# Kelvin-ywc/LPI

Hardware: AMD Instinct MI355X
Metric: image-text pairs/sec fwd+bwd (ViT-B/16, bs256/GPU) (higher is better)
Workload: dtype bf16; 1 GPU; BASELINE.json configs[2]: ViT-B/16 dual encoder bs=256/GPU prompt_depth=3 r=4 P=16, fwd+bwd incl. DecomposedPrompt grads + SGD step; global_batch=256, image=224x224, towers=lock step, GEMMs of one layer op grouped in one launch, parallelism=dp1, weights=synthetic (numpy Philox, CLIP-init scales), frozen

## Files before the change

lpi_amd/csrc/attention.hip:

```cpp
#include <type_traits>
#include "common.h"
#include "attn_softmax.h"

extern int g_lpi_tuning[16];

namespace {

constexpr int HD = 64;
constexpr int NB = 2;
constexpr float LOG2E = 1.4426950408889634f;
constexpr float LN2 = 0.6931471805599453f;
constexpr float SCALE = 0.125f;

template <typename T> struct AT;
template <> struct AT<float> {
    static constexpr int KS = 4;
    static constexpr int RS = 272;
};
template <> struct AT<f16_t> {
    static constexpr int KS = 2;
    static constexpr int RS = 160;
};
template <> struct AT<bf16_t> {
    static constexpr int KS = 2;
    static constexpr int RS = 160;
};

template <typename T, bool CV0 = false, bool CV1 = false, bool SW = false>
__device__ __forceinline__ void stage_rows2(char* lds0, const T* g0, char* lds1, const T* g1, int ld0, int ld1, int L, int Lp, int pre = 0, long seg = 0) {
    constexpr int NCH = HD * (int)sizeof(T) / 16;
    const int n = Lp * NCH, nt = blockDim.x;
    for (int base = threadIdx.x; base < n; base += 4 * nt) {
        uint4 v0[4], v1[4];
#pragma unroll
        for (int j = 0; j < 4; ++j) {
            const int i = base + j * nt, row = i / NCH, c = i % NCH;
            v0[j] = make_uint4(0, 0, 0, 0);
            v1[j] = make_uint4(0, 0, 0, 0);
            if (i < n && row < L) {
                const size_t srow = (size_t)(row < pre ? (long)row : (long)row + seg);
                v0[j] = *reinterpret_cast<const uint4*>(g0 + srow * ld0 + c * Elem<T>::EPC);
                v1[j] = *reinterpret_cast<const uint4*>(g1 + srow * ld1 + c * Elem<T>::EPC);
            }
        }
#pragma unroll
        for (int j = 0; j < 4; ++j) {
            const int i = base + j * nt, row = i / NCH, c = i % NCH;
            if (i < n) {
                if constexpr (CV0) { Chunk t; t.u = v0[j]; chunk_f16_to_bf16(t); v0[j] = t.u; }
                if constexpr (CV1) { Chunk t; t.u = v1[j]; chunk_f16_to_bf16(t); v1[j] = t.u; }
                const int lo = SW ? row * 128 + ((c ^ (row & 6)) << 4) : row * AT<T>::RS + c * 16;
                *reinterpret_cast<uint4*>(lds0 + lo) = v0[j];
                *reinterpret_cast<uint4*>(lds1 + lo) = v1[j];
            }
        }
    }
}

template <typename T, bool CVA>
__device__ __forceinline__ void stage_rows4(char* lds_k, const T* gk, char* lds_v, const T* gv, int ldkv, int La, int pre, long seg,
                                            char* lds_q, const T* gq, int ldq, char* lds_do, const T* gdo, int lddo, int Lb, int Lp) {
    constexpr int NCH = HD * (int)sizeof(T) / 16;
    const int n = Lp * NCH, nt = blockDim.x;
    for (int base = threadIdx.x; base < n; base += 4 * nt) {
        uint4 vk[4], vv[4], vq[4], vd[4];
#pragma unroll
        for (int j = 0; j < 4; ++j) {
            const int i = base + j * nt, row = i / NCH, c = i % NCH;
            vk[j] = vv[j] = vq[j] = vd[j] = make_uint4(0, 0, 0, 0);
            if (i < n && row < La) {
                const size_t srow = (size_t)(row < pre ? (long)row : (long)row + seg);
                vk[j] = *reinterpret_cast<const uint4*>(gk + srow * ldkv + c * Elem<T>::EPC);
                vv[j] = *reinterpret_cast<const uint4*>(gv + srow * ldkv + c * Elem<T>::EPC);
            }
            if (i < n && row < Lb) {
                vq[j] = *reinterpret_cast<const uint4*>(gq + (size_t)row * ldq + c * Elem<T>::EPC);
                vd[j] = *reinterpret_cast<const uint4*>(gdo + (size_t)row * lddo + c * Elem<T>::EPC);
            }
        }
#pragma unroll
        for (int j = 0; j < 4; ++j) {
            const int i = base + j * nt, row = i / NCH, c = i % NCH;
            if (i < n) {
                if constexpr (CVA) {
                    Chunk t;
                    t.u = vk[j]; chunk_f16_to_bf16(t); vk[j] = t.u;
                    t.u = vv[j]; chunk_f16_to_bf16(t); vv[j] = t.u;
                    t.u = vq[j]; chunk_f16_to_bf16(t); vq[j] = t.u;
                }
                const int lo = row * AT<T>::RS + c * 16;
                *reinterpret_cast<uint4*>(lds_k + lo) = vk[j];
                *reinterpret_cast<uint4*>(lds_v + lo) = vv[j];
                *reinterpret_cast<uint4*>(lds_q + lo) = vq[j];
                *reinterpret_cast<uint4*>(lds_do + lo) = vd[j];
            }
        }
    }
}

template <typename T>
__device__ __forceinline__ void lds_row_chunks(Chunk (&q)[AT<T>::KS], const char* lds, int row, int grp) {
#pragma unroll
    for (int ks = 0; ks < AT<T>::KS; ++ks) q[ks].u = *reinterpret_cast<const uint4*>(lds + row * AT<T>::RS + (grp + 4 * ks) * 16);
}

template <typename T, bool CV = false>
__device__ __forceinline__ void load_row_chunks(Chunk (&q)[AT<T>::KS], const T* g, size_t row, int ld, int grp, bool valid) {
#pragma unroll
    for (int ks = 0; ks < AT<T>::KS; ++ks) {
        q[ks].u = make_uint4(0, 0, 0, 0);
        if (valid) q[ks].u = *reinterpret_cast<const uint4*>(g + row * ld + (grp + 4 * ks) * Elem<T>::EPC);
        if constexpr (CV) chunk_f16_to_bf16(q[ks]);
    }
}

__device__ __forceinline__ float fast_exp2(float x) { return __builtin_amdgcn_exp2f(x); }

typedef __attribute__((ext_vector_type(2))) float f32x2;
typedef __attribute__((ext_vector_type(2))) __bf16 bf16x2;
__device__ __forceinline__ uint32_t pack_bf16(float a, float b) {
    return __builtin_bit_cast(uint32_t, __builtin_convertvector((f32x2){a, b}, bf16x2));
}

template <typename T>
__device__ __forceinline__ void mma_lds_rows(f32x4 (&acc)[NB], const char* p, const Chunk (&b)[NB][AT<T>::KS]) {
#pragma unroll
    for (int j = 0; j < NB; ++j) acc[j] = f32x4{0.f, 0.f, 0.f, 0.f};
#pragma unroll
    for (int ks = 0; ks < AT<T>::KS; ++ks) {
        Chunk a;
        a.u = *reinterpret_cast<const uint4*>(p + ks * 64);
#pragma unroll
        for (int j = 0; j < NB; ++j) mma_chunk<T>(acc[j], a, b[j][ks]);
    }
}

template <typename T>
__device__ __forceinline__ void mma_transposed(f32x4 (&acc)[NB][4], const char* tp, const f32x4 (&p0)[NB], const f32x4 (&p1)[NB]) {
    if constexpr (sizeof(T) == 2) {
        Chunk b[NB];
#pragma unroll
        for (int j = 0; j < NB; ++j)
            b[j].u = make_uint4(pack2_t<T>(p0[j][0], p0[j][1]), pack2_t<T>(p0[j][2], p0[j][3]), pack2_t<T>(p1[j][0], p1[j][1]), pack2_t<T>(p1[j][2], p1[j][3]));
#pragma unroll
        for (int dt = 0; dt < 4; ++dt) {
            short4v lo = __builtin_amdgcn_ds_read_tr16_b64_v4i16((__attribute__((address_space(3))) short4v*)(tp + dt * 32));
            short4v hi = __builtin_amdgcn_ds_read_tr16_b64_v4i16((__attribute__((address_space(3))) short4v*)(tp + 16 * AT<T>::RS + dt * 32));
            Chunk a;
            const uint2 lo2 = __builtin_bit_cast(uint2, lo), hi2 = __builtin_bit_cast(uint2, hi);
            a.u = make_uint4(lo2.x, lo2.y, hi2.x, hi2.y);
#pragma unroll
            for (int j = 0; j < NB; ++j) mma_chunk<T>(acc[j][dt], a, b[j]);
        }
    } else {
        const float* base = reinterpret_cast<const float*>(tp);
        constexpr int RSF = AT<T>::RS / 4;
#pragma unroll
        for (int dt = 0; dt < 4; ++dt) {
            Chunk a0, a1;
#pragma unroll
            for (int s = 0; s < 4; ++s) {
                a0.f[s] = base[s * RSF + dt * 16];
                a1.f[s] = base[(16 + s) * RSF + dt * 16];
            }
#pragma unroll
            for (int j = 0; j < NB; ++j) {
                Chunk b0, b1;
                b0.f = p0[j];
                b1.f = p1[j];
                mma_chunk<T>(acc[j][dt], a0, b0);
                mma_chunk<T>(acc[j][dt], a1, b1);
            }
        }
    }
}

template <typename T>
__device__ __forceinline__ void mma_lds_rows_sw(f32x4 (&acc)[NB], const char* base, const int (&ro)[AT<T>::KS], const Chunk (&b)[NB][AT<T>::KS]) {
#pragma unroll
    for (int j = 0; j < NB; ++j) acc[j] = f32x4{0.f, 0.f, 0.f, 0.f};
#pragma unroll
    for (int ks = 0; ks < AT<T>::KS; ++ks) {
        Chunk a;
        a.u = *reinterpret_cast<const uint4*>(base + ro[ks]);
#pragma unroll
        for (int j = 0; j < NB; ++j) mma_chunk<T>(acc[j], a, b[j][ks]);
    }
}
template <typename T>
__device__ __forceinline__ void mma_transposed_sw(f32x4 (&acc)[NB][4], const char* base, const int (&to)[4], const f32x4 (&p0)[NB], const f32x4 (&p1)[NB]) {
    Chunk b[NB];
#pragma unroll
    for (int j = 0; j < NB; ++j)
        b[j].u = make_uint4(pack2_t<T>(p0[j][0], p0[j][1]), pack2_t<T>(p0[j][2], p0[j][3]), pack2_t<T>(p1[j][0], p1[j][1]), pack2_t<T>(p1[j][2], p1[j][3]));
#pragma unroll
    for (int dt = 0; dt < 4; ++dt) {
        short4v lo = __builtin_amdgcn_ds_read_tr16_b64_v4i16((__attribute__((address_space(3))) short4v*)(base + to[dt]));
        short4v hi = __builtin_amdgcn_ds_read_tr16_b64_v4i16((__attribute__((address_space(3))) short4v*)(base + 16 * 128 + to[dt]));
        Chunk a;
        const uint2 lo2 = __builtin_bit_cast(uint2, lo), hi2 = __builtin_bit_cast(uint2, hi);
        a.u = make_uint4(lo2.x, lo2.y, hi2.x, hi2.y);
#pragma unroll
        for (int j = 0; j < NB; ++j) mma_chunk<T>(acc[j][dt], a, b[j]);
    }
}

template <typename T> __device__ __forceinline__ int row_ptr_off(int lane) { return (lane & 15) * AT<T>::RS + (lane >> 4) * 16; }
template <typename T> __device__ __forceinline__ int tr_ptr_off(int lane) {
    if constexpr (sizeof(T) == 2) return (4 * (lane >> 4) + ((lane & 15) >> 2)) * AT<T>::RS + (lane & 3) * 8;
    else return 4 * (lane >> 4) * AT<T>::RS + (lane & 15) * 4;
}

__device__ __forceinline__ float group_max(float v) {
    auto r = __builtin_amdgcn_permlane16_swap(__float_as_uint(v), __float_as_uint(v), false, false);
    v = fmaxf(__uint_as_float(r[0]), __uint_as_float(r[1]));
    r = __builtin_amdgcn_permlane32_swap(__float_as_uint(v), __float_as_uint(v), false, false);
    return fmaxf(__uint_as_float(r[0]), __uint_as_float(r[1]));
}
__device__ __forceinline__ float group_sum(float v) {
    auto r = __builtin_amdgcn_permlane16_swap(__float_as_uint(v), __float_as_uint(v), false, false);
    v = __uint_as_float(r[0]) + __uint_as_float(r[1]);
    r = __builtin_amdgcn_permlane32_swap(__float_as_uint(v), __float_as_uint(v), false, false);
    return __uint_as_float(r[0]) + __uint_as_float(r[1]);
}

template <typename T, bool CAUSAL, bool SW = false>
__device__ __forceinline__ void attn_fwd_body(int bh, char* smem, int Lmax, int Lpmax, const int* __restrict__ rs, int H, const T* __restrict__ qkv, int ldqkv,
                                              T* __restrict__ ctx, int ldctx, float* __restrict__ lse, int pre = 0, int bshared = -1,
                                              int qkv_hs = 0, int qkv_vs = 0, int ctx_hs = 0) {
    const int hs = qkv_hs ? qkv_hs : HD, chs = ctx_hs ? ctx_hs : HD;
    const int b = bh / H, h = bh % H;
    int L = Lmax, Lp = Lpmax;
    size_t row0 = (size_t)b * Lmax;
    int pb = 0;
    if (CAUSAL && pre > 0 && b == bshared) {
        row0 = 0;
        L = pre;
        Lp = (L + 31) / 32 * 32;
    } else if (rs) {
        const int r = rs[b];
        row0 = (size_t)r;
        L = rs[b + 1] - r;
        if (CAUSAL && pre > 0) pb = pre;
        Lp = (pb + L + 31) / 32 * 32;
    }
    const int Lk = pb + L;
    const size_t lse0 = ((size_t)b * H + h) * Lmax;
    const int dm = qkv_vs ? qkv_vs : H * HD;
    const T* qg = qkv + row0 * ldqkv + (size_t)h * hs;
    constexpr int RSX = SW ? 128 : AT<T>::RS;
    static_assert(!SW || sizeof(T) == 2, "the swizzled images are for the 2-byte operand types");
    char* k_lds = smem;
    char* v_lds = smem + Lp * RSX;
    const int lane = threadIdx.x & 63, wave = threadIdx.x >> 6, nw = blockDim.x >> 6;
    const int g = lane >> 4;
    Chunk q[NB][AT<T>::KS];
#pragma unroll
    for (int j = 0; j < NB; ++j) {
        const int qr = (wave * NB + j) * 16 + (lane & 15);
        load_row_chunks<T>(q[j], qg, qr, ldqkv, g, qr < L);
    }
    if (pb) stage_rows2<T, false, false, SW>(k_lds, qkv + (size_t)h * hs + dm, v_lds, qkv + (size_t)h * hs + 2 * (size_t)dm, ldqkv, ldqkv, Lk, Lp, pb, (long)row0 - pb);
    else stage_rows2<T, false, false, SW>(k_lds, qg + dm, v_lds, qg + 2 * (size_t)dm, ldqkv, ldqkv, L, Lp);
    __syncthreads();

    const float c = SCALE * LOG2E;
    const char* const kp0 = k_lds + row_ptr_off<T>(lane);
    const char* const vt0 = v_lds + tr_ptr_off<T>(lane);
    int ro[AT<T>::KS], to[4];
    {
        const int r = lane & 15, rr = 4 * g + (r >> 2), pq = lane & 3;
#pragma unroll
        for (int ks = 0; ks < AT<T>::KS; ++ks) ro[ks] = r * 128 + (((g + 4 * ks) ^ (r & 6)) << 4);
#pragma unroll
        for (int dt = 0; dt < 4; ++dt) to[dt] = rr * 128 + (((2 * dt + (pq >> 1)) ^ (rr & 6)) << 4) + (pq & 1) * 8;
    }
    for (int q0 = wave * 16 * NB; q0 < L; q0 += nw * 16 * NB) {
        int qrow[NB], qpos[NB];
#pragma unroll
        for (int j = 0; j < NB; ++j) { qrow[j] = q0 + 16 * j + (lane & 15); qpos[j] = qrow[j] + pb; }
        if (q0 != wave * 16 * NB) {
#pragma unroll
            for (int j = 0; j < NB; ++j) load_row_chunks<T>(q[j], qg, qrow[j], ldqkv, g, qrow[j] < L);
        }
        float m[NB], lsum[NB];
        f32x4 o[NB][4];
#pragma unroll
        for (int j = 0; j < NB; ++j) {
            m[j] = -INFINITY;
            lsum[j] = 0.f;
#pragma unroll
            for (int i = 0; i < 4; ++i) o[j][i] = f32x4{0.f, 0.f, 0.f, 0.f};
        }
        auto tile = [&](int kb, auto masked_tag) {
            constexpr bool MASKED = decltype(masked_tag)::value;
            f32x4 s0[NB], s1[NB];
            if constexpr (SW) {
                const char* kb_ = k_lds + kb * 128;
                mma_lds_rows_sw<T>(s0, kb_, ro, q);
                mma_lds_rows_sw<T>(s1, kb_ + 16 * 128, ro, q);
                attn_softmax_tile<NB, MASKED, CAUSAL>(s0, s1, m, lsum, o, kb, g, Lk, qpos, c);
                mma_transposed_sw<T>(o, v_lds + kb * 128, to, s0, s1);
            } else {
                const char* kp = kp0 + kb * AT<T>::RS;
                mma_lds_rows<T>(s0, kp, q);
                mma_lds_rows<T>(s1, kp + 16 * AT<T>::RS, q);
                attn_softmax_tile<NB, MASKED, CAUSAL>(s0, s1, m, lsum, o, kb, g, Lk, qpos, c);
                mma_transposed<T>(o, vt0 + kb * AT<T>::RS, s0, s1);
            }
        };
        const int qlast = q0 + pb + 16 * NB - 1;
        const int kend = CAUSAL ? min(Lp, (qlast / 32 + 1) * 32) : Lp;
        const int kfull = CAUSAL ? min((Lk / 32) * 32, ((q0 + pb) / 32) * 32) : (Lk / 32) * 32;
        int kb = 0;
        for (; kb < kfull; kb += 32) tile(kb, std::false_type{});
        for (; kb < kend; kb += 32) tile(kb, std::true_type{});
#pragma unroll
        for (int j = 0; j < NB; ++j) {
            const float ltot = group_sum(lsum[j]);
            const float inv = 1.0f / ltot;
            if constexpr (sizeof(T) == 2) {
                f32x4 os[4];
#pragma unroll
                for (int dt = 0; dt < 4; ++dt) os[dt] = o[j][dt] * inv;
                store_row16_t<T>(ctx + (row0 + qrow[j]) * ldctx + (size_t)h * chs, os, g, qrow[j] < L);
                if (qrow[j] < L && g == 0) lse[lse0 + qrow[j]] = (m[j] + log2f(ltot)) * LN2;
            } else if (qrow[j] < L) {
                T* dst = ctx + (row0 + qrow[j]) * ldctx + (size_t)h * chs + 4 * g;
#pragma unroll
                for (int dt = 0; dt < 4; ++dt) Elem<T>::st4(dst + dt * 16, o[j][dt] * inv);
                if (g == 0) lse[lse0 + qrow[j]] = (m[j] + log2f(ltot)) * LN2;
            }
        }
    }
}

template <typename T, bool CAUSAL, bool SW = false>
__global__ __launch_bounds__(512) void attn_fwd_kernel(int Lmax, int Lpmax, const int* __restrict__ rs, int H, const T* __restrict__ qkv, int ldqkv,
                                                      T* __restrict__ ctx, int ldctx, float* __restrict__ lse, int pre, int bshared, int hs, int vs, int chs) {
    extern __shared__ __attribute__((aligned(16))) char smem[];
    attn_fwd_body<T, CAUSAL, SW>(blockIdx.x, smem, Lmax, Lpmax, rs, H, qkv, ldqkv, ctx, ldctx, lse, pre, bshared, hs, vs, chs);
}
template <typename T>
struct AttnFwdP {
    int L, Lp, H, ldqkv, ldctx;
    const int* rs; const T* qkv; T* ctx; float* lse;
    int pre, bshared;
    int hs, vs, chs;
};
template <typename T, bool C0, bool C1, bool SW0 = false>
__global__ __launch_bounds__(512) void attn_fwd_pair_kernel(AttnFwdP<T> p0, AttnFwdP<T> p1, int nb0) {
    extern __shared__ __attribute__((aligned(16))) char smem[];
    if ((int)blockIdx.x < nb0) attn_fwd_body<T, C0, SW0>(blockIdx.x, smem, p0.L, p0.Lp, p0.rs, p0.H, p0.qkv, p0.ldqkv, p0.ctx, p0.ldctx, p0.lse, p0.pre, p0.bshared, p0.hs, p0.vs, p0.chs);
    else attn_fwd_body<T, C1>(blockIdx.x - nb0, smem, p1.L, p1.Lp, p1.rs, p1.H, p1.qkv, p1.ldqkv, p1.ctx, p1.ldctx, p1.lse, p1.pre, p1.bshared, p1.hs, p1.vs, p1.chs);
}

template <typename T, bool CAUSAL, bool SV16 = false>
__global__ __launch_bounds__(512) void attn_bwd_dq_kernel(int Lmax, int Lpmax, const int* __restrict__ rs, int H, const T* __restrict__ qkv, int ldqkv,
                                                         const T* __restrict__ ctx, int ldctx, const T* __restrict__ dctx, int lddctx,
                                                         const float* __restrict__ lse, float* __restrict__ delta,
                                                         T* __restrict__ dqkv, int lddqkv, int pre, int bshared, int q_hs, int q_vs, int dq_hs, int dq_vs) {
    extern __shared__ __attribute__((aligned(16))) char smem[];
    const int b = blockIdx.x / H, h = blockIdx.x % H;
    int L = Lmax, Lp = Lpmax;
    size_t row0 = (size_t)b * Lmax;
    int pb = 0;
    if (CAUSAL && pre > 0 && b == bshared) {
        row0 = 0;
        L = pre;
        Lp = (L + 31) / 32 * 32;
    } else if (rs) {
        const int r = rs[b];
        row0 = (size_t)r;
        L = rs[b + 1] - r;
        if (CAUSAL && pre > 0) pb = pre;
        Lp = (pb + L + 31) / 32 * 32;
    }
    const int Lk = pb + L;
    const size_t lse0 = ((size_t)b * H + h) * Lmax;
    const int hsq = q_hs ? q_hs : HD, vsq = q_vs ? q_vs : H * HD, hsd = dq_hs ? dq_hs : HD, vsd = dq_vs ? dq_vs : H * HD;
    const T* qg = qkv + row0 * ldqkv + (size_t)h * hsq;
    char* k_lds = smem;
    char* v_lds = smem + Lp * AT<T>::RS;
    if (pb) stage_rows2<T, SV16, SV16>(k_lds, qkv + (size_t)h * hsq + vsq, v_lds, qkv + (size_t)h * hsq + 2 * (size_t)vsq, ldqkv, ldqkv, Lk, Lp, pb, (long)row0 - pb);
    else stage_rows2<T, SV16, SV16>(k_lds, qg + vsq, v_lds, qg + 2 * (size_t)vsq, ldqkv, ldqkv, L, Lp);
    __syncthreads();

    const int lane = threadIdx.x & 63, wave = threadIdx.x >> 6, nw = blockDim.x >> 6;
    const int g = lane >> 4;
    const float c = SCALE * LOG2E;
    const char* const kp0 = k_lds + row_ptr_off<T>(lane);
    const char* const vp0 = v_lds + row_ptr_off<T>(lane);
    const char* const kt0 = k_lds + tr_ptr_off<T>(lane);
    for (int q0 = wave * 16 * NB; q0 < L; q0 += nw * 16 * NB) {
        int qrow[NB];
        Chunk q[NB][AT<T>::KS], dO[NB][AT<T>::KS];
        float dls[NB], lq[NB];
        f32x4 dq[NB][4];
#pragma unroll
        for (int j = 0; j < NB; ++j) {
            qrow[j] = q0 + 16 * j + (lane & 15);
            const bool valid = qrow[j] < L;
            const size_t grow = row0 + qrow[j];
            load_row_chunks<T, SV16>(q[j], qg, qrow[j], ldqkv, g, valid);
            load_row_chunks<T>(dO[j], dctx + h * HD, grow, lddctx, g, valid);
            Chunk oc[AT<T>::KS];
            load_row_chunks<T>(oc, ctx + h * HD, grow, ldctx, g, valid);
            float dl = 0.f;
#pragma unroll
            for (int ks = 0; ks < AT<T>::KS; ++ks) {
                if constexpr (sizeof(T) == 4) {
#pragma unroll
                    for (int e = 0; e < 4; ++e) dl += oc[ks].f[e] * dO[j][ks].f[e];
                } else {
#pragma unroll
                    for (int e = 0; e < 8; ++e) dl += (SV16 ? (float)oc[ks].hh[e] : (float)oc[ks].h[e]) * (float)dO[j][ks].h[e];
                }
            }
            dl = group_sum(dl);
            lq[j] = valid ? lse[lse0 + qrow[j]] * LOG2E : INFINITY;
            if (valid && g == 0) delta[lse0 + qrow[j]] = dl;
            dls[j] = dl * SCALE;
#pragma unroll
            for (int i = 0; i < 4; ++i) dq[j][i] = f32x4{0.f, 0.f, 0.f, 0.f};
        }
        auto tile = [&](int kb, auto masked_tag) {
            constexpr bool MASKED = decltype(masked_tag)::value;
            const char* kp = kp0 + kb * AT<T>::RS;
            const char* vp = vp0 + kb * AT<T>::RS;
            f32x4 s0[NB], s1[NB], p0[NB], p1[NB];
            mma_lds_rows<T>(s0, kp, q);
            mma_lds_rows<T>(s1, kp + 16 * AT<T>::RS, q);
            mma_lds_rows<T>(p0, vp, dO);
            mma_lds_rows<T>(p1, vp + 16 * AT<T>::RS, dO);
#pragma unroll
            for (int j = 0; j < NB; ++j)
#pragma unroll
                for (int r = 0; r < 4; ++r) {
                    float e0 = fast_exp2(fmaf(s0[j][r], c, -lq[j]));
                    float e1 = fast_exp2(fmaf(s1[j][r], c, -lq[j]));
                    if constexpr (MASKED) {
                        const int k0 = kb + 4 * g + r, k1 = k0 + 16;
                        if (!(k0 < Lk && (!CAUSAL || k0 <= qrow[j] + pb))) e0 = 0.f;
                        if (!(k1 < Lk && (!CAUSAL || k1 <= qrow[j] + pb))) e1 = 0.f;
                    }
                    s0[j][r] = e0 * fmaf(p0[j][r], SCALE, -dls[j]);
                    s1[j][r] = e1 * fmaf(p1[j][r], SCALE, -dls[j]);
                }
            mma_transposed<T>(dq, kt0 + kb * AT<T>::RS, s0, s1);
        };
        const int qlast = q0 + pb + 16 * NB - 1;
        const int kend = CAUSAL ? min(Lp, (qlast / 32 + 1) * 32) : Lp;
        const int kfull = CAUSAL ? min((Lk / 32) * 32, ((q0 + pb) / 32) * 32) : (Lk / 32) * 32;
        int kb = 0;
        for (; kb < kfull; kb += 32) tile(kb, std::false_type{});
        for (; kb < kend; kb += 32) tile(kb, std::true_type{});
#pragma unroll
        for (int j = 0; j < NB; ++j) {
            if constexpr (sizeof(T) == 2) {
                store_row_bf16_t(reinterpret_cast<bf16_t*>(dqkv) + (row0 + qrow[j]) * lddqkv + (size_t)h * hsd, dq[j], g, qrow[j] < L);
            } else if (qrow[j] < L) {
                T* dst = dqkv + (row0 + qrow[j]) * lddqkv + (size_t)h * hsd + 4 * g;
#pragma unroll
                for (int dt = 0; dt < 4; ++dt) Elem<T>::st4(dst + dt * 16, dq[j][dt]);
            }
        }
    }
}

template <typename T, bool CAUSAL, bool SV16 = false>
__global__ __launch_bounds__(512) void attn_bwd_dkv_kernel(int Lmax, int Lpmax, const int* __restrict__ rs, int H, const T* __restrict__ qkv, int ldqkv,
                                                          const T* __restrict__ dctx, int lddctx, const float* __restrict__ lse,
                                                          const float* __restrict__ delta, T* __restrict__ dqkv, int lddqkv, int pre, int bshared,
                                                          float* __restrict__ shared_dkv, int q_hs, int q_vs, int dq_hs, int dq_vs) {
    extern __shared__ __attribute__((aligned(16))) char smem[];
    const int b = blockIdx.x / H, h = blockIdx.x % H;
    int L = Lmax, Lp = Lpmax;
    size_t row0 = (size_t)b * Lmax;
    int pb = 0;
    if (CAUSAL && pre > 0 && b == bshared) {
        row0 = 0;
        L = pre;
        Lp = (L + 31) / 32 * 32;
    } else if (rs) {
        const int r = rs[b];
// ... 215 lines not shown
#pragma unroll
            for (int i = 0; i < 4; ++i) dq[j][i] = f32x4{0.f, 0.f, 0.f, 0.f};
        }
        auto tile = [&](int kb, auto masked_tag) {
            constexpr bool MASKED = decltype(masked_tag)::value;
            f32x4 s0[NB], s1[NB], p0[NB], p1[NB];
            mma_lds_rows<T>(s0, kp0 + kb * AT<T>::RS, q);
            mma_lds_rows<T>(s1, kp0 + (kb + 16) * AT<T>::RS, q);
            mma_lds_rows<T>(p0, vp0 + kb * AT<T>::RS, dO);
            mma_lds_rows<T>(p1, vp0 + (kb + 16) * AT<T>::RS, dO);
#pragma unroll
            for (int j = 0; j < NB; ++j)
#pragma unroll
                for (int r = 0; r < 4; ++r) {
                    float e0 = fast_exp2(fmaf(s0[j][r], c, -lq[j]));
                    float e1 = fast_exp2(fmaf(s1[j][r], c, -lq[j]));
                    if constexpr (MASKED) {
                        const int k0 = kb + 4 * g + r, k1 = k0 + 16;
                        if (!(k0 < Lk && (!CAUSAL || k0 <= qrow[j] + pb))) e0 = 0.f;
                        if (!(k1 < Lk && (!CAUSAL || k1 <= qrow[j] + pb))) e1 = 0.f;
                    }
                    s0[j][r] = e0 * fmaf(p0[j][r], SCALE, -dls[j]);
                    s1[j][r] = e1 * fmaf(p1[j][r], SCALE, -dls[j]);
                }
            mma_transposed<T>(dq, kt0 + kb * AT<T>::RS, s0, s1);
        };
        if (q0 + pb >= rows_hi) continue;
        const int qlast = q0 + pb + 16 * NB - 1;
        const int kend = CAUSAL ? min(Lp, (qlast / 32 + 1) * 32) : Lp;
        const int kfull = CAUSAL ? min((Lk / 32) * 32, ((q0 + pb) / 32) * 32) : (Lk / 32) * 32;
        int kb = 0;
        for (; kb < kfull; kb += 32) tile(kb, std::false_type{});
        for (; kb < kend; kb += 32) tile(kb, std::true_type{});
#pragma unroll
        for (int j = 0; j < NB; ++j) {
            if constexpr (sizeof(T) == 2) {
                store_row_bf16_t(reinterpret_cast<bf16_t*>(dqkv) + (row0 + qrow[j]) * lddqkv + (size_t)h * hsd, dq[j], g, qrow[j] < L);
            } else if (qrow[j] < L) {
                T* dst = dqkv + (row0 + qrow[j]) * lddqkv + (size_t)h * hsd + 4 * g;
#pragma unroll
                for (int dt = 0; dt < 4; ++dt) Elem<T>::st4(dst + dt * 16, dq[j][dt]);
            }
        }
    }
    __syncthreads();

    for (int k0 = wave * 16 * NB; k0 < min(Lk, rows_hi); k0 += nw * 16 * NB) {
        int krow[NB];
        Chunk kk[NB][AT<T>::KS], vv[NB][AT<T>::KS];
        f32x4 dk[NB][4], dv[NB][4];
#pragma unroll
        for (int j = 0; j < NB; ++j) {
            krow[j] = k0 + 16 * j + (lane & 15);
            lds_row_chunks<T>(kk[j], k_lds, krow[j], g);
            lds_row_chunks<T>(vv[j], v_lds, krow[j], g);
#pragma unroll
            for (int i = 0; i < 4; ++i) { dk[j][i] = f32x4{0.f, 0.f, 0.f, 0.f}; dv[j][i] = f32x4{0.f, 0.f, 0.f, 0.f}; }
        }
        auto tile = [&](int qb, auto masked_tag) {
            constexpr bool MASKED = decltype(masked_tag)::value;
            f32x4 s0[NB], s1[NB], p0[NB], p1[NB], e0[NB], e1[NB];
            mma_lds_rows<T>(s0, qp0 + qb * AT<T>::RS, kk);
            mma_lds_rows<T>(s1, qp0 + (qb + 16) * AT<T>::RS, kk);
            mma_lds_rows<T>(p0, dp0 + qb * AT<T>::RS, vv);
            mma_lds_rows<T>(p1, dp0 + (qb + 16) * AT<T>::RS, vv);
            const f32x4 l0 = *reinterpret_cast<const f32x4*>(lse_lds + qb + 4 * g);
            const f32x4 l1 = *reinterpret_cast<const f32x4*>(lse_lds + qb + 16 + 4 * g);
            const f32x4 d0 = *reinterpret_cast<const f32x4*>(dl_lds + qb + 4 * g);
            const f32x4 d1 = *reinterpret_cast<const f32x4*>(dl_lds + qb + 16 + 4 * g);
#pragma unroll
            for (int j = 0; j < NB; ++j)
#pragma unroll
                for (int r = 0; r < 4; ++r) {
                    e0[j][r] = fast_exp2(fmaf(s0[j][r], c, -l0[r]));
                    e1[j][r] = fast_exp2(fmaf(s1[j][r], c, -l1[r]));
                    if constexpr (MASKED) {
                        const int qa = qb + pb + 4 * g + r, qc = qa + 16;
                        if (krow[j] > qa) e0[j][r] = 0.f;
                        if (krow[j] > qc) e1[j][r] = 0.f;
                    }
                    s0[j][r] = e0[j][r] * fmaf(p0[j][r], SCALE, -d0[r]);
                    s1[j][r] = e1[j][r] * fmaf(p1[j][r], SCALE, -d1[r]);
                }
            mma_transposed<T>(dv, dt0 + qb * AT<T>::RS, e0, e1);
            mma_transposed<T>(dk, qt0 + qb * AT<T>::RS, s0, s1);
        };
        const int kq = k0 - pb;
        int qb = CAUSAL ? (kq > 0 ? (kq / 32) * 32 : 0) : 0;
        if constexpr (CAUSAL) {
            const int qdiag = (kq + 16 * NB - 1 >= 0) ? min(Lp, ((kq + 16 * NB - 1) / 32 + 1) * 32) : 0;
            for (; qb < qdiag; qb += 32) tile(qb, std::true_type{});
        }
        for (; qb < Lp; qb += 32) tile(qb, std::false_type{});
#pragma unroll
        for (int j = 0; j < NB; ++j) {
            if (pb && krow[j] < pb) {
                float* dst = shared_dkv + ((size_t)b * pb + krow[j]) * 2 * dm + h * HD + 4 * g;
#pragma unroll
                for (int dt = 0; dt < 4; ++dt) {
                    *reinterpret_cast<f32x4*>(dst + dt * 16) = dk[j][dt];
                    *reinterpret_cast<f32x4*>(dst + dm + dt * 16) = dv[j][dt];
                }
                continue;
            }
            const size_t orow = row0 + (krow[j] - pb);
            if constexpr (sizeof(T) == 2) {
                bf16_t* dst = reinterpret_cast<bf16_t*>(dqkv) + orow * lddqkv + (size_t)h * hsd;
                store_row_bf16_t(dst + vsd, dk[j], g, krow[j] < Lk);
                store_row_bf16_t(dst + 2 * (size_t)vsd, dv[j], g, krow[j] < Lk);
            } else if (krow[j] < Lk) {
                T* dst = dqkv + orow * lddqkv + (size_t)h * hsd + 4 * g;
#pragma unroll
                for (int dt = 0; dt < 4; ++dt) {
                    Elem<T>::st4(dst + vsd + dt * 16, dk[j][dt]);
                    Elem<T>::st4(dst + 2 * (size_t)vsd + dt * 16, dv[j][dt]);
                }
            }
        }
    }
}

inline int pick_waves(int L) {
    const int nqb = (L + 16 * NB - 1) / (16 * NB);
    const int rounds = (nqb + 7) / 8;
    return (nqb + rounds - 1) / rounds;
}
inline int pick_waves_ragged(int L) {
    const int w = pick_waves(L), lo = g_lpi_tuning[9];
    return lo > w ? (lo < 8 ? lo : 8) : w;
}

int set_lds(const void* kern, size_t bytes) {
    if (bytes > 160 * 1024) return LPI_EINVAL;
    static const void* fn[32];
    static LdsOnce once[32];
    static std::atomic<int> nfn{0};
    static std::atomic_flag lock = ATOMIC_FLAG_INIT;
    int slot = -1;
    const int n = nfn.load(std::memory_order_acquire);
    for (int i = 0; i < n; ++i)
        if (fn[i] == kern) { slot = i; break; }
    if (slot < 0) {
        while (lock.test_and_set(std::memory_order_acquire)) {}
        const int m = nfn.load(std::memory_order_relaxed);
        for (int i = 0; i < m; ++i)
            if (fn[i] == kern) { slot = i; break; }
        if (slot < 0 && m < 32) { fn[m] = kern; slot = m; nfn.store(m + 1, std::memory_order_release); }
        lock.clear(std::memory_order_release);
    }
    if (slot < 0) return (int)hipFuncSetAttribute(kern, hipFuncAttributeMaxDynamicSharedMemorySize, 160 * 1024);
    return lpi_ensure_lds(once[slot], kern, 160 * 1024);
}

static bool fwd_swizzled(int Lp) { return g_lpi_tuning[13] != 1 && (size_t)2 * 2 * Lp * 160 > (size_t)160 * 1024 && (size_t)2 * 2 * Lp * 128 <= (size_t)160 * 1024; }

template <typename T, bool CAUSAL>
int fwd_launch(int B, int L, int H, const void* qkv, int ldqkv, void* ctx, int ldctx, float* lse, hipStream_t s, const int* rs = nullptr, int pre = 0,
               int hs = 0, int vs = 0, int chs = 0) {
    const int nbh = (B + (pre > 0 ? 1 : 0)) * H, bsh = pre > 0 ? B : -1;
    const int Lp = (L + 31) / 32 * 32;
    const size_t lds = (size_t)2 * Lp * AT<T>::RS;
    const int thr = 64 * (rs ? pick_waves_ragged(L) : pick_waves(L));
    if constexpr (sizeof(T) == 2 && !CAUSAL) {
        if (fwd_swizzled(Lp) && !rs) {
            const size_t lsw = (size_t)2 * Lp * 128;
            if (int e = set_lds((const void*)attn_fwd_kernel<T, CAUSAL, true>, lsw)) return e;
            LPI_LAUNCH((attn_fwd_kernel<T, CAUSAL, true>), dim3(nbh), dim3(thr), lsw, s, L, Lp, rs, H, (const T*)qkv, ldqkv, (T*)ctx, ldctx, lse, pre, bsh, hs, vs, chs);
            LPI_CHECK_LAST();
            return 0;
        }
    }
    int e = set_lds((const void*)attn_fwd_kernel<T, CAUSAL>, lds);
    if (e) return e;
    LPI_LAUNCH((attn_fwd_kernel<T, CAUSAL>), dim3(nbh), dim3(thr), lds, s, L, Lp, rs, H, (const T*)qkv, ldqkv, (T*)ctx, ldctx, lse, pre, bsh, hs, vs, chs);
    LPI_CHECK_LAST();
    return 0;
}

template <typename T, bool CAUSAL, bool SV16 = false>
int bwd_launch(int B, int L, int H, const void* qkv, int ldqkv, const void* ctx, int ldctx, const void* dctx, int lddctx,
               const float* lse, float* delta, void* dqkv, int lddqkv, hipStream_t s, const int* rs = nullptr, int rows_hi = 1 << 30, int pre = 0,
               float* shared_dkv = nullptr, const int* lay = nullptr) {
    const int l0 = lay ? lay[0] : 0, l1 = lay ? lay[1] : 0, l2 = lay ? lay[2] : 0, l3 = lay ? lay[3] : 0;
    const int Lp = (L + 31) / 32 * 32;
    const size_t ldsA = (size_t)2 * Lp * AT<T>::RS;
    const size_t ldsB = ldsA + (size_t)2 * Lp * sizeof(float);
    const int thr = 64 * (rs ? pick_waves_ragged(L) : pick_waves(L));
    const size_t ldsF = (size_t)4 * Lp * AT<T>::RS + (size_t)2 * Lp * sizeof(float);
    if (sizeof(T) == 2 && ldsF <= 160 * 1024 && g_lpi_tuning[3] == 0) {
        int ef = set_lds((const void*)attn_bwd_fused_kernel<T, CAUSAL, SV16>, ldsF);
        if (ef) return ef;
        LPI_LAUNCH((attn_bwd_fused_kernel<T, CAUSAL, SV16>), dim3((B + (pre > 0 ? 1 : 0)) * H), dim3(thr), ldsF, s, L, Lp, rs, H, (const T*)qkv, ldqkv,
                   (const T*)ctx, ldctx, (const T*)dctx, lddctx, lse, delta, (T*)dqkv, lddqkv, rows_hi, pre, pre > 0 ? B : -1, shared_dkv, l0, l1, l2, l3);
        LPI_CHECK_LAST();
        return 0;
    }
    int e = set_lds((const void*)attn_bwd_dq_kernel<T, CAUSAL, SV16>, ldsA);
    if (e) return e;
    e = set_lds((const void*)attn_bwd_dkv_kernel<T, CAUSAL, SV16>, ldsB);
    if (e) return e;
    const int nbh = (B + (pre > 0 ? 1 : 0)) * H, bsh = pre > 0 ? B : -1;
    LPI_LAUNCH((attn_bwd_dq_kernel<T, CAUSAL, SV16>), dim3(nbh), dim3(thr), ldsA, s, L, Lp, rs, H, (const T*)qkv, ldqkv, (const T*)ctx, ldctx,
               (const T*)dctx, lddctx, lse, delta, (T*)dqkv, lddqkv, pre, bsh, l0, l1, l2, l3);
    LPI_CHECK_LAST();
    LPI_LAUNCH((attn_bwd_dkv_kernel<T, CAUSAL, SV16>), dim3(nbh), dim3(thr), ldsB, s, L, Lp, rs, H, (const T*)qkv, ldqkv, (const T*)dctx, lddctx,
               lse, delta, (T*)dqkv, lddqkv, pre, bsh, shared_dkv, l0, l1, l2, l3);
    LPI_CHECK_LAST();
    return 0;
}

inline bool bad_attn(int dtype, int B, int L, int H, int ld, int lmax = 288) {
    const int esz = dtype == LPI_F32 ? 4 : 2;
    return B <= 0 || H <= 0 || L <= 0 || L > lmax || ld < 3 * H * HD || (ld * esz) % 16;
}

}

bool lpi_attn_long_ok(int L, int causal, const void* row_start);
int lpi_attn_long_fwd(int dtype, int B, int L, int H, const void* qkv, int ldqkv, void* ctx, int ldctx, float* lse, hipStream_t s);
int lpi_attn_long_bwd(int dtype, int B, int L, int H, const void* qkv, int ldqkv, const void* ctx, int ldctx, const void* dctx, int lddctx, const float* lse,
                      float* delta, void* dqkv, int lddqkv, hipStream_t s);

bool lpi_attn4_bwd_ok(int L, int causal);
int lpi_attn4_bwd(int B, int L, int H, const void* qkv, int ldqkv, const void* ctx, int ldctx, const void* dctx, int lddctx, const float* lse,
                  float* delta, void* dqkv, int lddqkv, hipStream_t s, int saved_f16, int rows_hi, const int* lay = nullptr);
extern "C" int lpi_attn_fwd_varlen(int dtype, int B, int L, const int32_t* row_start, int H, const void* qkv, int ldqkv, void* ctx, int ldctx,
                                   float* lse, int causal, void* stream) {
    const int* rs = row_start;
    const bool lng = lpi_attn_long_ok(L, causal, row_start);
    if (!qkv || !ctx || !lse || bad_attn(dtype, B, L, H, ldqkv, lng ? 1024 : 288) || ldctx < H * HD || (ldctx & 7)) return LPI_EINVAL;
    if (((uintptr_t)qkv | (uintptr_t)ctx) & 15) return LPI_EINVAL;
    hipStream_t s = (hipStream_t)stream;
    if (lng) return lpi_attn_long_fwd(dtype, B, L, H, qkv, ldqkv, ctx, ldctx, lse, s);
    if (dtype == LPI_F32)
        return causal ? fwd_launch<float, true>(B, L, H, qkv, ldqkv, ctx, ldctx, lse, s, rs) : fwd_launch<float, false>(B, L, H, qkv, ldqkv, ctx, ldctx, lse, s, rs);
    if (dtype == LPI_F16)
        return causal ? fwd_launch<f16_t, true>(B, L, H, qkv, ldqkv, ctx, ldctx, lse, s, rs) : fwd_launch<f16_t, false>(B, L, H, qkv, ldqkv, ctx, ldctx, lse, s, rs);
    if (dtype == LPI_BF16) {
        return causal ? fwd_launch<bf16_t, true>(B, L, H, qkv, ldqkv, ctx, ldctx, lse, s, rs) : fwd_launch<bf16_t, false>(B, L, H, qkv, ldqkv, ctx, ldctx, lse, s, rs);
    }
    return LPI_EINVAL;
}

extern "C" int lpi_attn_fwd(int dtype, int B, int L, int H, const void* qkv, int ldqkv, void* ctx, int ldctx, float* lse, int causal,
                            void* stream) {
    return lpi_attn_fwd_varlen(dtype, B, L, nullptr, H, qkv, ldqkv, ctx, ldctx, lse, causal, stream);
}

template <typename T>
static int fwd_pair_launch(const lpi_attn_fwd_desc* d, hipStream_t s) {
    AttnFwdP<T> p[2];
    size_t lds = 0;
    int thr = 0;
    for (int i = 0; i < 2; ++i) {
        const int Lp = (d[i].L + 31) / 32 * 32;
        const int pre = d[i].shared_rows;
        if (pre < 0 || (pre > 0 && (!d[i].causal || !d[i].row_start || pre >= d[i].L))) return LPI_EINVAL;
        p[i] = AttnFwdP<T>{d[i].L, Lp, d[i].H, d[i].ldqkv, d[i].ldctx, d[i].row_start, (const T*)d[i].qkv, (T*)d[i].ctx, d[i].lse, pre, pre > 0 ? d[i].B : -1,
                           d[i].qkv_hs, d[i].qkv_vs, d[i].ctx_hs};
        lds = std::max(lds, (size_t)2 * Lp * AT<T>::RS);
        thr = std::max(thr, 64 * (d[i].row_start ? pick_waves_ragged(d[i].L) : pick_waves(d[i].L)));
    }
    const int nb0 = (d[0].B + (d[0].shared_rows > 0)) * d[0].H, nb1 = (d[1].B + (d[1].shared_rows > 0)) * d[1].H;
    if (!d[0].causal && d[1].causal && !d[0].row_start && fwd_swizzled(p[0].Lp)) {
        const size_t lsw = std::max((size_t)2 * p[0].Lp * 128, (size_t)2 * p[1].Lp * AT<T>::RS);
        if (int e = set_lds((const void*)attn_fwd_pair_kernel<T, false, true, true>, lsw)) return e;
        LPI_LAUNCH((attn_fwd_pair_kernel<T, false, true, true>), dim3(nb0 + nb1), dim3(thr), lsw, s, p[0], p[1], nb0);
        LPI_CHECK_LAST();
        return 0;
    }
#define FP(C0, C1)                                                                                                              \
    do {                                                                                                                        \
        if (int e = set_lds((const void*)attn_fwd_pair_kernel<T, C0, C1>, lds)) return e;                                       \
        LPI_LAUNCH((attn_fwd_pair_kernel<T, C0, C1>), dim3(nb0 + nb1), dim3(thr), lds, s, p[0], p[1], nb0);                     \
    } while (0)
    if (d[0].causal && d[1].causal) FP(true, true);
    else if (d[0].causal) FP(true, false);
    else if (d[1].causal) FP(false, true);
    else FP(false, false);
#undef FP
    LPI_CHECK_LAST();
    return 0;
}
extern "C" int lpi_attn_fwd_varlen(int dtype, int B, int L, const int32_t* row_start, int H, const void* qkv, int ldqkv, void* ctx, int ldctx,
                                   float* lse, int causal, void* stream);
extern "C" int lpi_attn_fwd_pair(int dtype, const lpi_attn_fwd_desc* d, void* stream) {
    if (!d) return LPI_EINVAL;
    bool any_long = false;
    for (int i = 0; i < 2; ++i) {
        const bool lay = d[i].qkv_hs || d[i].qkv_vs || d[i].ctx_hs;
        if (lay && (dtype == LPI_F32 || d[i].row_start || d[i].shared_rows || !d[i].qkv_hs || !d[i].qkv_vs || !d[i].ctx_hs ||
                    ((d[i].qkv_hs | d[i].qkv_vs | d[i].ctx_hs | d[i].ldqkv | d[i].ldctx) & 7) || d[i].ldqkv < HD || d[i].ldctx < HD)) return LPI_EINVAL;
        const bool lng = !lay && !d[i].shared_rows && lpi_attn_long_ok(d[i].L, d[i].causal, d[i].row_start);
        any_long |= lng;
        if (!d[i].qkv || !d[i].ctx || !d[i].lse || (!lay && (bad_attn(dtype, d[i].B, d[i].L, d[i].H, d[i].ldqkv, lng ? 1024 : 288) || d[i].ldctx < d[i].H * HD)) || (d[i].ldctx & 7))
            return LPI_EINVAL;
        if (lay && (d[i].B <= 0 || d[i].H <= 0 || d[i].L <= 0 || d[i].L > 288)) return LPI_EINVAL;
        if (((uintptr_t)d[i].qkv | (uintptr_t)d[i].ctx) & 15) return LPI_EINVAL;
    }
    if (dtype == LPI_BF16 && !any_long) return fwd_pair_launch<bf16_t>(d, (hipStream_t)stream);
    if (dtype == LPI_F16 && !any_long) return fwd_pair_launch<f16_t>(d, (hipStream_t)stream);
    for (int i = 0; i < 2; ++i) {
        if (d[i].shared_rows) {
            if (int e = lpi_attn_fwd_shared(dtype, d[i].B, d[i].L, d[i].row_start, d[i].shared_rows, d[i].H, d[i].qkv, d[i].ldqkv, d[i].ctx, d[i].ldctx, d[i].lse, stream)) return e;
            continue;
        }
        if (int e = lpi_attn_fwd_varlen(dtype, d[i].B, d[i].L, d[i].row_start, d[i].H, d[i].qkv, d[i].ldqkv, d[i].ctx, d[i].ldctx, d[i].lse, d[i].causal, stream))
            return e;
    }
    return 0;
}

namespace {
template <typename T>
__global__ __launch_bounds__(256) void shared_kv_reduce_kernel(int B, int pre, int dm, const float* __restrict__ part, T* __restrict__ dqkv, int ld, int accumulate) {
    __shared__ f32x4 red[16][16];
    const int per_row = 2 * dm / 4, n = pre * per_row;
    const int o = threadIdx.x & 15, slice = threadIdx.x >> 4;
    const int t = blockIdx.x * 16 + o;
    f32x4 a = {0.f, 0.f, 0.f, 0.f};
    if (t < n) {
        const int key = t / per_row, c = (t % per_row) * 4;
        const float* p = part + (size_t)key * 2 * dm + c;
        const size_t bstride = (size_t)pre * 2 * dm;
        f32x4 a1 = a;
        int b = slice;
        for (; b + 16 < B; b += 32) {
            a += *reinterpret_cast<const f32x4*>(p + (size_t)b * bstride);
            a1 += *reinterpret_cast<const f32x4*>(p + (size_t)(b + 16) * bstride);
        }
        if (b < B) a += *reinterpret_cast<const f32x4*>(p + (size_t)b * bstride);
        a += a1;
    }
    red[slice][o] = a;
    __syncthreads();
    if (slice == 0 && t < n) {
        f32x4 v = red[0][o];
#pragma unroll
        for (int i = 1; i < 16; ++i) v += red[i][o];
        const int key = t / per_row, c = (t % per_row) * 4;
        T* out = dqkv + (size_t)key * ld + dm + c;
        if (accumulate) v += Elem<T>::ld4(out);
        Elem<T>::st4(out, v);
    }
}
}

extern "C" int lpi_shared_kv_reduce(int dtype, int B, int shared_rows, int H, const float* partial, void* dqkv, int lddqkv, int accumulate, void* stream) {
    if (!partial || !dqkv || B <= 0 || shared_rows <= 0 || H <= 0 || lddqkv < 3 * H * HD || (lddqkv & 3) || ((uintptr_t)partial & 15) || ((uintptr_t)dqkv & (dtype == LPI_F32 ? 15 : 7))) return LPI_EINVAL;
    const int dm = H * HD, n = shared_rows * (2 * dm / 4);
    hipStream_t s = (hipStream_t)stream;
    if (dtype == LPI_BF16 || dtype == LPI_F16)
        LPI_LAUNCH((shared_kv_reduce_kernel<bf16_t>), dim3((n + 15) / 16), dim3(256), 0, s, B, shared_rows, dm, partial, (bf16_t*)dqkv, lddqkv, accumulate);
    else if (dtype == LPI_F32)
        LPI_LAUNCH((shared_kv_reduce_kernel<float>), dim3((n + 15) / 16), dim3(256), 0, s, B, shared_rows, dm, partial, (float*)dqkv, lddqkv, accumulate);
    else
        return LPI_ENOSYS;
    LPI_CHECK_LAST();
    return 0;
}

extern "C" int lpi_attn_fwd_shared(int dtype, int B, int L, const int32_t* row_start, int shared_rows, int H, const void* qkv, int ldqkv, void* ctx, int ldctx,
                                   float* lse, void* stream) {
    if (!qkv || !ctx || !lse || !row_start || shared_rows <= 0 || shared_rows >= L || bad_attn(dtype, B, L, H, ldqkv) || ldctx < H * HD || (ldctx & 7)) return LPI_EINVAL;
    if (((uintptr_t)qkv | (uintptr_t)ctx) & 15) return LPI_EINVAL;
    hipStream_t s = (hipStream_t)stream;
    if (dtype == LPI_F16) return fwd_launch<f16_t, true>(B, L, H, qkv, ldqkv, ctx, ldctx, lse, s, row_start, shared_rows);
    if (dtype == LPI_BF16) return fwd_launch<bf16_t, true>(B, L, H, qkv, ldqkv, ctx, ldctx, lse, s, row_start, shared_rows);
    if (dtype == LPI_F32) return fwd_launch<float, true>(B, L, H, qkv, ldqkv, ctx, ldctx, lse, s, row_start, shared_rows);
    return LPI_ENOSYS;
}

extern "C" int lpi_attn_bwd_shared(int dtype, int B, int L, const int32_t* row_start, int shared_rows, int rows_needed, int H, const void* qkv, int ldqkv,
                                   const void* ctx, int ldctx, const void* dctx, int lddctx, const float* lse, float* delta, void* dqkv, int lddqkv,
                                   float* shared_dkv, void* stream) {
    if (!row_start || !shared_dkv || shared_rows <= 0 || shared_rows >= L || rows_needed < shared_rows) return LPI_EINVAL;
    const int rows_hi = rows_needed >= L ? (1 << 30) : rows_needed;
    if (!qkv || !ctx || !dctx || !lse || !delta || !dqkv || bad_attn(dtype, B, L, H, ldqkv) || bad_attn(dtype, B, L, H, lddqkv)) return LPI_EINVAL;
    const int esz = dtype == LPI_F32 ? 4 : 2;
    if (ldctx < H * HD || lddctx < H * HD || (ldctx * esz) % 16 || (lddctx * esz) % 16) return LPI_EINVAL;
    if (((uintptr_t)qkv | (uintptr_t)ctx | (uintptr_t)dctx | (uintptr_t)dqkv | (uintptr_t)shared_dkv) & 15) return LPI_EINVAL;
    hipStream_t s = (hipStream_t)stream;
    int e;
    if (dtype == LPI_F32)
        e = bwd_launch<float, true>(B, L, H, qkv, ldqkv, ctx, ldctx, dctx, lddctx, lse, delta, dqkv, lddqkv, s, row_start, rows_hi, shared_rows, shared_dkv);
    else if (dtype == LPI_F16) e = bwd_launch<bf16_t, true, true>(B, L, H, qkv, ldqkv, ctx, ldctx, dctx, lddctx, lse, delta, dqkv, lddqkv, s, row_start, rows_hi, shared_rows, shared_dkv);
    else if (dtype == LPI_BF16) e = bwd_launch<bf16_t, true>(B, L, H, qkv, ldqkv, ctx, ldctx, dctx, lddctx, lse, delta, dqkv, lddqkv, s, row_start, rows_hi, shared_rows, shared_dkv);
    else return LPI_ENOSYS;
    if (e) return e;
    return lpi_shared_kv_reduce(dtype, B, shared_rows, H, shared_dkv, dqkv, lddqkv, 1, stream);
}

extern "C" int lpi_attn_bwd_prefix(int dtype, int B, int L, const int32_t* row_start, int rows_needed, int H, const void* qkv, int ldqkv, const void* ctx,
                                   int ldctx, const void* dctx, int lddctx, const float* lse, float* delta, void* dqkv, int lddqkv, int causal,
                                   void* stream) {
    const int* rs = row_start;
    if (rows_needed <= 0) return LPI_EINVAL;
    const int rows_hi = rows_needed >= L ? (1 << 30) : rows_needed;
    const bool lng = lpi_attn_long_ok(L, causal, row_start);
    const int lmax = lng ? 1024 : 288;
    if (!qkv || !ctx || !dctx || !lse || !delta || !dqkv || bad_attn(dtype, B, L, H, ldqkv, lmax) || bad_attn(dtype, B, L, H, lddqkv, lmax)) return LPI_EINVAL;
    const int esz = dtype == LPI_F32 ? 4 : 2;
    if (ldctx < H * HD || lddctx < H * HD || (ldctx * esz) % 16 || (lddctx * esz) % 16) return LPI_EINVAL;
    if (((uintptr_t)qkv | (uintptr_t)ctx | (uintptr_t)dctx | (uintptr_t)dqkv) & 15) return LPI_EINVAL;
    hipStream_t s = (hipStream_t)stream;
    if (lng) return lpi_attn_long_bwd(dtype, B, L, H, qkv, ldqkv, ctx, ldctx, dctx, lddctx, lse, delta, dqkv, lddqkv, s);
    if (dtype == LPI_F32)
        return causal ? bwd_launch<float, true>(B, L, H, qkv, ldqkv, ctx, ldctx, dctx, lddctx, lse, delta, dqkv, lddqkv, s, rs, rows_hi)
                      : bwd_launch<float, false>(B, L, H, qkv, ldqkv, ctx, ldctx, dctx, lddctx, lse, delta, dqkv, lddqkv, s, rs, rows_hi);
    if (dtype == LPI_F16) {
        if (!rs && g_lpi_tuning[3] == 0 && lpi_attn4_bwd_ok(L, causal) && (g_lpi_tuning[7] == 5 || (g_lpi_tuning[7] == 0 && L > 160)))
            return lpi_attn4_bwd(B, L, H, qkv, ldqkv, ctx, ldctx, dctx, lddctx, lse, delta, dqkv, lddqkv, s, 1, rows_hi);
        return causal ? bwd_launch<bf16_t, true, true>(B, L, H, qkv, ldqkv, ctx, ldctx, dctx, lddctx, lse, delta, dqkv, lddqkv, s, rs, rows_hi)
                      : bwd_launch<bf16_t, false, true>(B, L, H, qkv, ldqkv, ctx, ldctx, dctx, lddctx, lse, delta, dqkv, lddqkv, s, rs, rows_hi);
    }
    if (dtype == LPI_BF16) {
        if (!rs && g_lpi_tuning[3] == 0 && lpi_attn4_bwd_ok(L, causal) && (g_lpi_tuning[7] == 5 || (g_lpi_tuning[7] == 0 && L > 160)))
// ... 50 lines not shown
```

Before: 11850 pairs/s.

## Stage swizzled forward K/V via global-to-LDS DMA with progressive waits

In the swizzled non-causal forward attention path, K and V rows are now copied straight from global memory into LDS with global_load_lds_dwordx4, replacing the register round-trip through stage_rows2. Each wave waits only for the tiles it needs before each PV tile (vmcnt plus a barrier), so the first QK^T tiles can overlap the remaining staging. The swizzle selector also drops its lower-bound LDS condition, so more sequence lengths (including ViT's L=197+prompts) take the swizzled path, guarded by a 32-bit offset limit. This relies on hand-counted vmcnt bookkeeping and inline asm that sets M0, which is fragile.

```diff
diff --git a/lpi_amd/csrc/attention.hip b/lpi_amd/csrc/attention.hip
--- a/lpi_amd/csrc/attention.hip
+++ b/lpi_amd/csrc/attention.hip
@@ -26,7 +26,7 @@
     static constexpr int RS = 160;
 };
 
-template <typename T, bool CV0 = false, bool CV1 = false, bool SW = false>
+template <typename T, bool CV0 = false, bool CV1 = false>
 __device__ __forceinline__ void stage_rows2(char* lds0, const T* g0, char* lds1, const T* g1, int ld0, int ld1, int L, int Lp, int pre = 0, long seg = 0) {
     constexpr int NCH = HD * (int)sizeof(T) / 16;
     const int n = Lp * NCH, nt = blockDim.x;
@@ -49,12 +49,38 @@
             if (i < n) {
                 if constexpr (CV0) { Chunk t; t.u = v0[j]; chunk_f16_to_bf16(t); v0[j] = t.u; }
                 if constexpr (CV1) { Chunk t; t.u = v1[j]; chunk_f16_to_bf16(t); v1[j] = t.u; }
-                const int lo = SW ? row * 128 + ((c ^ (row & 6)) << 4) : row * AT<T>::RS + c * 16;
+                const int lo = row * AT<T>::RS + c * 16;
                 *reinterpret_cast<uint4*>(lds0 + lo) = v0[j];
                 *reinterpret_cast<uint4*>(lds1 + lo) = v1[j];
             }
         }
     }
+}
+
+__device__ __forceinline__ void fwd_glds16s(const void* sbase, unsigned voff, unsigned lds_addr) {
+    unsigned keep;
+    asm volatile("s_mov_b32 %0, m0\n\ts_mov_b32 m0, %3\n\ts_nop 0\n\tglobal_load_lds_dwordx4 %1, %2\n\ts_mov_b32 m0, %0"
+                 : "=&s"(keep) : "v"(voff), "s"(sbase), "s"(__builtin_amdgcn_readfirstlane(lds_addr)) : "memory");
+}
+__device__ __forceinline__ const void* fwd_scalar_ptr(const void* p) {
+    const unsigned long long a = (unsigned long long)p;
+    const unsigned lo = __builtin_amdgcn_readfirstlane((unsigned)a), hi = __builtin_amdgcn_readfirstlane((unsigned)(a >> 32));
+    return (const void*)(((unsigned long long)hi << 32) | lo);
+}
+template <int N> __device__ __forceinline__ void vmcnt_le() { asm volatile("s_waitcnt vmcnt(%0)" ::"n"(N) : "memory"); }
+__device__ __forceinline__ void vm_wait(int n) {
+    switch (n) {
+#define LPI_VMW(N) case N: vmcnt_le<N>(); break;
+        LPI_VMW(0) LPI_VMW(1) LPI_VMW(2) LPI_VMW(3) LPI_VMW(4) LPI_VMW(5) LPI_VMW(6) LPI_VMW(7)
+        LPI_VMW(8) LPI_VMW(9) LPI_VMW(10) LPI_VMW(11) LPI_VMW(12) LPI_VMW(13) LPI_VMW(14)
+#undef LPI_VMW
+        default: vmcnt_le<15>(); break;
+    }
+}
+__device__ __forceinline__ void lds_barrier() {
+    asm volatile("s_waitcnt lgkmcnt(0)" ::: "memory");
+    __builtin_amdgcn_s_barrier();
+    asm volatile("" ::: "memory");
 }
 
 template <typename T, bool CVA>
@@ -255,14 +281,58 @@
     const int lane = threadIdx.x & 63, wave = threadIdx.x >> 6, nw = blockDim.x >> 6;
     const int g = lane >> 4;
     Chunk q[NB][AT<T>::KS];
-#pragma unroll
-    for (int j = 0; j < NB; ++j) {
-        const int qr = (wave * NB + j) * 16 + (lane & 15);
-        load_row_chunks<T>(q[j], qg, qr, ldqkv, g, qr < L);
-    }
-    if (pb) stage_rows2<T, false, false, SW>(k_lds, qkv + (size_t)h * hs + dm, v_lds, qkv + (size_t)h * hs + 2 * (size_t)dm, ldqkv, ldqkv, Lk, Lp, pb, (long)row0 - pb);
-    else stage_rows2<T, false, false, SW>(k_lds, qg + dm, v_lds, qg + 2 * (size_t)dm, ldqkv, ldqkv, L, Lp);
-    __syncthreads();
+    static_assert(!SW || (!CAUSAL && NB == 2 && AT<T>::KS == 2), "the DMA staging is the non-causal 2-byte body");
+    const int wv = __builtin_amdgcn_readfirstlane(wave);
+    const int npc = 8 * (Lp >> 5);
+    auto dma_left = [&](int t) {
+        const int tot = wv < npc ? (npc - wv + nw - 1) / nw : 0, j0 = t <= wv ? 0 : (t - wv + nw - 1) / nw;
+        return tot > j0 ? tot - j0 : 0;
+    };
+    auto q_issue = [&](int q0) {
+#pragma unroll
+        for (int j = 0; j < NB; ++j) {
+            const int qr = q0 + 16 * j + (lane & 15);
+#pragma unroll
+            for (int ks = 0; ks < AT<T>::KS; ++ks) {
+                const T* src = qg + (size_t)min(qr, L - 1) * ldqkv + (g + 4 * ks) * Elem<T>::EPC;
+                asm volatile("global_load_dwordx4 %0, %1, off" : "=v"(q[j][ks].f) : "v"(src) : "memory");
+            }
+        }
+    };
+    auto q_fix = [&](int q0) {
+        asm volatile("" : "+v"(q[0][0].f), "+v"(q[0][1].f), "+v"(q[1][0].f), "+v"(q[1][1].f));
+#pragma unroll
+        for (int j = 0; j < NB; ++j) {
+            const int qr = q0 + 16 * j + (lane & 15);
+#pragma unroll
+            for (int ks = 0; ks < AT<T>::KS; ++ks)
+                if (qr >= L) q[j][ks].u = make_uint4(0, 0, 0, 0);
+        }
+    };
+    if constexpr (SW) {
+        q_issue(wv * 16 * NB);
+        const unsigned lds0 = __builtin_amdgcn_readfirstlane((unsigned)(uintptr_t)(__attribute__((address_space(3))) char*)smem);
+        const void* const kbase = fwd_scalar_ptr(qg + dm);
+        const void* const vbase = fwd_scalar_ptr(qg + 2 * (size_t)dm);
+        for (int p = wv; p < npc; p += nw) {
+            const int i = p & 7, r0 = 32 * (p >> 3) + 8 * (i & 3), row = r0 + (lane >> 3);
+            const unsigned voff = (unsigned)(min(row, L - 1) * ldqkv + (((lane & 7) ^ (row & 6)) << 3)) * (unsigned)sizeof(T);
+            fwd_glds16s(i < 4 ? kbase : vbase, voff, lds0 + (i < 4 ? 0u : (unsigned)(Lp * 128)) + (unsigned)(r0 * 128));
+        }
+        vm_wait(dma_left(4));
+        lds_barrier();
+        q_fix(wv * 16 * NB);
+    } else {
+#pragma unroll
+        for (int j = 0; j < NB; ++j) {
+            const int qr = (wave * NB + j) * 16 + (lane & 15);
+            load_row_chunks<T>(q[j], qg, qr, ldqkv, g, qr < L);
+        }
+        if (pb) stage_rows2<T>(k_lds, qkv + (size_t)h * hs + dm, v_lds, qkv + (size_t)h * hs + 2 * (size_t)dm, ldqkv, ldqkv, Lk, Lp, pb, (long)row0 - pb);
+        else stage_rows2<T>(k_lds, qg + dm, v_lds, qg + 2 * (size_t)dm, ldqkv, ldqkv, L, Lp);
+        __syncthreads();
+    }
+    int vw = 0;
 
     const float c = SCALE * LOG2E;
     const char* const kp0 = k_lds + row_ptr_off<T>(lane);
@@ -280,8 +350,14 @@
 #pragma unroll
         for (int j = 0; j < NB; ++j) { qrow[j] = q0 + 16 * j + (lane & 15); qpos[j] = qrow[j] + pb; }
         if (q0 != wave * 16 * NB) {
-#pragma unroll
-            for (int j = 0; j < NB; ++j) load_row_chunks<T>(q[j], qg, qrow[j], ldqkv, g, qrow[j] < L);
+            if constexpr (SW) {
+                q_issue(q0);
+                vmcnt_le<0>();
+                q_fix(q0);
+            } else {
+#pragma unroll
+                for (int j = 0; j < NB; ++j) load_row_chunks<T>(q[j], qg, qrow[j], ldqkv, g, qrow[j] < L);
+            }
         }
         float m[NB], lsum[NB];
         f32x4 o[NB][4];
@@ -300,6 +376,11 @@
                 mma_lds_rows_sw<T>(s0, kb_, ro, q);
                 mma_lds_rows_sw<T>(s1, kb_ + 16 * 128, ro, q);
                 attn_softmax_tile<NB, MASKED, CAUSAL>(s0, s1, m, lsum, o, kb, g, Lk, qpos, c);
+                if (kb >= vw) {
+                    vm_wait(dma_left(min(kb / 4 + 12, npc)));
+                    lds_barrier();
+                    vw = kb + 32;
+                }
                 mma_transposed_sw<T>(o, v_lds + kb * 128, to, s0, s1);
             } else {
                 const char* kp = kp0 + kb * AT<T>::RS;
@@ -331,6 +412,12 @@
                 for (int dt = 0; dt < 4; ++dt) Elem<T>::st4(dst + dt * 16, o[j][dt] * inv);
                 if (g == 0) lse[lse0 + qrow[j]] = (m[j] + log2f(ltot)) * LN2;
             }
+        }
+    }
+    if constexpr (SW) {
+        for (; vw < Lp; vw += 32) {
+            vm_wait(dma_left(min(vw / 4 + 12, npc)));
+            lds_barrier();
         }
     }
 }
@@ -852,7 +939,9 @@
     return lpi_ensure_lds(once[slot], kern, 160 * 1024);
 }
 
-static bool fwd_swizzled(int Lp) { return g_lpi_tuning[13] != 1 && (size_t)2 * 2 * Lp * 160 > (size_t)160 * 1024 && (size_t)2 * 2 * Lp * 128 <= (size_t)160 * 1024; }
+static bool fwd_swizzled(int Lp, int ldqkv) {
+    return g_lpi_tuning[13] != 1 && (size_t)2 * 2 * Lp * 128 <= (size_t)160 * 1024 && (size_t)Lp * (size_t)ldqkv * 2 < ((size_t)1 << 31);
+}
 
 template <typename T, bool CAUSAL>
 int fwd_launch(int B, int L, int H, const void* qkv, int ldqkv, void* ctx, int ldctx, float* lse, hipStream_t s, const int* rs = nullptr, int pre = 0,
@@ -862,7 +951,7 @@
     const size_t lds = (size_t)2 * Lp * AT<T>::RS;
     const int thr = 64 * (rs ? pick_waves_ragged(L) : pick_waves(L));
     if constexpr (sizeof(T) == 2 && !CAUSAL) {
-        if (fwd_swizzled(Lp) && !rs) {
+        if (fwd_swizzled(Lp, ldqkv) && !rs) {
             const size_t lsw = (size_t)2 * Lp * 128;
             if (int e = set_lds((const void*)attn_fwd_kernel<T, CAUSAL, true>, lsw)) return e;
             LPI_LAUNCH((attn_fwd_kernel<T, CAUSAL, true>), dim3(nbh), dim3(thr), lsw, s, L, Lp, rs, H, (const T*)qkv, ldqkv, (T*)ctx, ldctx, lse, pre, bsh, hs, vs, chs);
@@ -962,7 +1051,7 @@
         thr = std::max(thr, 64 * (d[i].row_start ? pick_waves_ragged(d[i].L) : pick_waves(d[i].L)));
     }
     const int nb0 = (d[0].B + (d[0].shared_rows > 0)) * d[0].H, nb1 = (d[1].B + (d[1].shared_rows > 0)) * d[1].H;
-    if (!d[0].causal && d[1].causal && !d[0].row_start && fwd_swizzled(p[0].Lp)) {
+    if (!d[0].causal && d[1].causal && !d[0].row_start && fwd_swizzled(p[0].Lp, p[0].ldqkv)) {
         const size_t lsw = std::max((size_t)2 * p[0].Lp * 128, (size_t)2 * p[1].Lp * AT<T>::RS);
         if (int e = set_lds((const void*)attn_fwd_pair_kernel<T, false, true, true>, lsw)) return e;
         LPI_LAUNCH((attn_fwd_pair_kernel<T, false, true, true>), dim3(nb0 + nb1), dim3(thr), lsw, s, p[0], p[1], nb0);
```

Result: no change. 11770 pairs/s (median of 2 runs) (-0.7%).
